# modelstreaming/ams

Measured on AMD Instinct MI355X. Metric: frames/sec student infer (DeeplabV3+MobileNetV2, 512x1024) + distill-steps/sec, higher is better.
Workload: dtype f32 (2xfp16 split products)

## Files before the change

ams_amd/csrc/api.hip:

```cpp
#include "engine.hpp"
#include "head_common.hpp"
#include "entry_check.hpp"

using namespace ams;

extern "C" {

const char* ams_last_error(void) { return ams::last_error(); }
int ams_abi_version(void) { return AMS_ABI_VERSION; }

int ams_device_info(char* name_out, size_t name_cap, int32_t* n_cu, int64_t* hbm_bytes) {
    int dev = 0;
    AMS_CHECK_HIP(hipGetDevice(&dev));
    hipDeviceProp_t p;
    AMS_CHECK_HIP(hipGetDeviceProperties(&p, dev));
    if (name_out && name_cap) { snprintf(name_out, name_cap, "%s (%s)", p.name, p.gcnArchName); }
    if (n_cu) *n_cu = p.multiProcessorCount;
    if (hbm_bytes) *hbm_bytes = (int64_t)p.totalGlobalMem;
    return AMS_OK;
}

int ams_student_arena_bytes(const ams_student_config* cfg, const ams_layer_desc* layers, size_t* bytes_out) {
    AMS_REQUIRE(bytes_out, "arena_bytes: null output");
    ams_student tmp;
// ... 1084 lines not shown
    const bool f32 = !f16 && Cin <= 32;
    const bool wreg = !f32 && presplit == 2;
    BlockCall c;
    c.B = B; c.H = H; c.W = W; c.Cin = Cin; c.Cexp = Cexp; c.rate = rate;
    if (f32 && rate < 0) { c.stride = -rate; c.rate = 1; }
    AMS_REQUIRE(B > 0 && H > 0 && W > 0, "expand_dw_steps: no pixels: B=%d, %d x %d", B, H, W);
    AMS_REQUIRE(expand_dw_stream_supported(Cin, Cexp, c.stride, c.rate) && (!f16 || Cin >= 64), "expand_dw_steps: unsupported shape Cin=%d Cexp=%d rate=%d",
                Cin, Cexp, rate);
    AMS_REQUIRE(out && n >= 10, "expand_dw_steps: out needs at least 10 elements");
    const int np = f32 ? 0 : (f16 ? 2 : 3);
    XdwGeom g;
    const bool fits = wreg ? expand_dw_wreg_geom(B, H, W, Cin, Cexp, c.rate, np, &g) : expand_dw_stream_geom(B, H, W, Cin, Cexp, c.rate, np, &g);
    AMS_REQUIRE(fits, "expand_dw_steps: no segment geometry fits LDS (W=%d rate=%d)", W, rate);
    expand_dw_steps(g, H, W, c.rate, out, n);
    return AMS_OK;
}

int ams_k_global_mean(const float* x, int32_t B, int64_t HW, int32_t C, float* y, float* scratch, size_t scratch_floats,
                      void* stream) {
    AMS_REQUIRE(scratch && scratch_floats >= image_colsum_scratch(B, C), "global_mean: scratch too small (need %zu floats)",
                image_colsum_scratch(B, C));
    return launch_global_mean(x, B, HW, C, y, scratch, (hipStream_t)stream);
}
size_t ams_k_global_mean_scratch(int32_t B, int32_t C) { return image_colsum_scratch(B, C); }

int ams_k_upsample_argmax(const float* logits, int32_t B, int32_t h, int32_t w, int32_t NC, const int32_t* class_idx_host, int32_t K,
                          int32_t H, int32_t W, const uint8_t* teacher, int32_t* labels_out, int64_t* conf_mat, double* loss,
                          void* stream) {
    const HeadCall c{logits, NC, B, h, w, class_idx_host, K, H, W, teacher, NC};
    return launch_upsample_argmax(c, labels_out, conf_mat, loss, (hipStream_t)stream);
// ... 599 lines not shown
```

ams_amd/csrc/k_block.hip:

```cpp
#include <type_traits>

#include "pw_common.hpp"
#include "split_bf16.hpp"
#include "block_call.hpp"

namespace ams {

struct BlkArgs {
    const float* x;
    int B, H, W, Cin;
    const float* w_exp;
    const float* sc_e; const float* sh_e;
    int Cexp;
    const float* w_dw;
    const float* sc_d; const float* sh_d;
    const float* w_pj;
    const float* sc_p; const float* sh_p;
    int Cout;
    int act_e, act_d, act_p, residual;
    float* y;
    int Ho, Wo, pt, pl;
    int tiles_x, tiles_y, chunks;
    const float* vecs;
    int fH, fW, spt, spl;
    float ps;
    const uint16_t* wparts;
    int64_t wplane;
    const uint16_t* he; int64_t he_plane;
    const uint16_t* hp; int64_t hp_plane; int kp_p;
    int timed;
};

__device__ unsigned long long g_blk_cycles[1024][8];

template <typename TIn>
__device__ __forceinline__ float blk_frame_value(const TIn* img, int H, int W, int iy, int ix, int ch, float ps) {
    const bool inside = iy >= 0 && ix >= 0 && iy <= H && ix <= W;
// ... 16 lines not shown

template <int S, int KC, int NTO, int TH, int TW, typename TIn = void, bool X6 = false, bool H16 = false, bool HP = H16>
__global__ __launch_bounds__(256, 2) void block_kernel(BlkArgs a, unsigned ntiles) {
    static_assert(!HP || H16, "HP is a refinement of H16");
    constexpr bool PKDW = S == 1 || TH == 2;
    constexpr bool SLIDE = S == 1 && TW == 16 && TH % 2 == 0;
    constexpr bool STEM = !std::is_void<TIn>::value;
    static_assert(!(X6 && STEM) && !(H16 && STEM) && !(X6 && H16), "the stem stays exact f32; one split form at a time");
    constexpr bool H16W = H16 && KC == 2;
    constexpr int IH = (TH - 1) * S + 3, IW = (TW - 1) * S + 3;
    constexpr int NPIX = IH * IW;
    constexpr int NRG = (NPIX + 15) / 16;
    constexpr int AP = blk_act_pitch(S, TW);
    constexpr int MRO = TH * TW / 16;
    static_assert(TH * TW % 16 == 0, "whole output row groups");
    extern __shared__ __attribute__((aligned(16))) float smem[];
    float* sVec = smem;
    const int tid = threadIdx.x, wave = __builtin_amdgcn_readfirstlane(tid >> 6), lane = tid & 63, l15 = lane & 15, q = lane >> 4;
    float* sAct = smem + 13 * a.Cexp + wave * (NRG * 16 * AP);
    unsigned long long tc[4] = {0, 0, 0, 0}, tl_ = a.timed ? __builtin_amdgcn_s_memtime() : 0;
    auto lap = [&](int slot) {
        if (a.timed) {
            const unsigned long long now = __builtin_amdgcn_s_memtime();
            tc[slot] += now - tl_;
            tl_ = now;
        }
    };

    if (a.vecs) {
        for (int e = tid; e < 13 * a.Cexp / 4; e += 256) st4(sVec + 4 * e, ld4(a.vecs + 4 * e));
    } else {
        for (int e = tid; e < 13 * a.Cexp; e += 256) {
            const int which = e / a.Cexp, c = e - which * a.Cexp;
            const float* src = which == 0 ? a.sc_e : which == 1 ? a.sh_e : which == 2 ? a.sc_d : which == 3 ? a.sh_d : a.w_dw + (which - 4) * a.Cexp;
            sVec[e] = src[c];
        }
    }
    unsigned wt = xcd_remap(blockIdx.x, gridDim.x) * 4 + wave;
    const bool live = wt < ntiles;
    if (!live) wt = ntiles - 1;
    const int tx = wt % a.tiles_x;
    unsigned t1 = wt / a.tiles_x;
    const int ty = t1 % a.tiles_y;
    const int b = t1 / a.tiles_y;
    const int oy0 = ty * TH, ox0 = tx * TW;
    const int iy0 = oy0 * S - a.pt, ix0 = ox0 * S - a.pl;

    const float lo_e = a.act_e == AMS_ACT_NONE ? -__builtin_huge_valf() : 0.f, hi_e = a.act_e == AMS_ACT_RELU6 ? 6.f : __builtin_huge_valf();
    const float lo_d = a.act_d == AMS_ACT_NONE ? -__builtin_huge_valf() : 0.f, hi_d = a.act_d == AMS_ACT_RELU6 ? 6.f : __builtin_huge_valf();
    const float* xb = STEM ? nullptr : a.x + (int64_t)b * a.H * a.W * a.Cin;
    float4 areg[(X6 || H16) ? 1 : NRG][KC];
    bf16x8 xp[X6 ? NRG : 1][3];
    u32x4 xh8[H16W ? NRG : 1], xl8[H16W ? NRG : 1];
    u32x2_t xh4[(H16 && !H16W) ? NRG : 1], xl4[(H16 && !H16W) ? NRG : 1];
    unsigned inside_mask = 0;
    if constexpr (STEM) {
        typedef typename std::conditional<STEM, TIn, float>::type TI;
        const TI* img = reinterpret_cast<const TI*>(a.x) + (int64_t)b * a.fH * a.fW * 3;
        int toff[KC][4], tdy[KC][4], tdx[KC][4], tch[KC][4];
#pragma unroll
        for (int c = 0; c < KC; ++c)
// ... 28 lines not shown
                for (int c = 0; c < KC; ++c)
#pragma unroll
                    for (int j = 0; j < 4; ++j)
                        t[c][j] = blk_frame_value(img, a.fH, a.fW, fy + tdy[c][j], fx + tdx[c][j], tch[c][j] < 0 ? 0 : tch[c][j], a.ps);
            }
#pragma unroll
            for (int c = 0; c < KC; ++c)
                areg[rg][c] = make_float4(tch[c][0] >= 0 ? t[c][0] : 0.f, tch[c][1] >= 0 ? t[c][1] : 0.f, tch[c][2] >= 0 ? t[c][2] : 0.f,
                                          tch[c][3] >= 0 ? t[c][3] : 0.f);
        }
    } else {
#pragma unroll
    for (int rg = 0; rg < NRG; ++rg) {
        const int m = rg * 16 + l15;
        const int ty_i = m / IW, tx_i = m - ty_i * IW;
        const int iy = iy0 + ty_i, ix = ix0 + tx_i;
        if (m < NPIX && iy >= 0 && iy < a.H && ix >= 0 && ix < a.W) inside_mask |= 1u << rg;
        const int iyc = iy < 0 ? 0 : (iy > a.H - 1 ? a.H - 1 : iy), ixc = ix < 0 ? 0 : (ix > a.W - 1 ? a.W - 1 : ix);
        const float* px = xb + ((int64_t)iyc * a.W + ixc) * a.Cin;
        if constexpr (X6 || H16W) {
            int k0 = 8 * q, k1 = 8 * q + 4;
            const bool ok0 = k0 < a.Cin, ok1 = k1 < a.Cin;
            if (k0 > a.Cin - 4) k0 = a.Cin - 4;
            if (k1 > a.Cin - 4) k1 = a.Cin - 4;
            float4 u = ld4(px + k0), v = ld4(px + k1);
            u = make_float4(ok0 ? u.x : 0.f, ok0 ? u.y : 0.f, ok0 ? u.z : 0.f, ok0 ? u.w : 0.f);
            v = make_float4(ok1 ? v.x : 0.f, ok1 ? v.y : 0.f, ok1 ? v.z : 0.f, ok1 ? v.w : 0.f);
            if constexpr (X6) split8(u, v, xp[rg][0], xp[rg][1], xp[rg][2]);
            else {
                f16x8 h, l;
                split8_f16(u, v, h, l);
                xh8[rg] = __builtin_bit_cast(u32x4, h); xl8[rg] = __builtin_bit_cast(u32x4, l);
            }
        } else if constexpr (H16) {
// ... 82 lines not shown
#pragma unroll
        for (int t = 0; t < NTO; ++t) out[i][t] = (f32x4){0.f, 0.f, 0.f, 0.f};
#pragma unroll
    for (int i = 0; i < (HP ? MRO : 1); ++i)
#pragma unroll
        for (int t = 0; t < (HP ? NTO : 1); ++t) outx[i][t] = (f32x4){0.f, 0.f, 0.f, 0.f};
    __syncthreads();
    lap(0);

    const int chunks = a.Cexp / 16;
    for (int ci = 0; ci < chunks; ++ci) {
        const int n0 = ci * 16;
        const int n_next = ci + 1 < chunks ? n0 + 16 : n0;
        {
            const float4 sc = ld4(sVec + n0 + 4 * q), sh = ld4(sVec + a.Cexp + n0 + 4 * q);
#pragma unroll
            for (int rg = 0; rg < NRG; ++rg) {
                f32x4 acc = (f32x4){0.f, 0.f, 0.f, 0.f};
                if constexpr (X6) {
                    acc = __builtin_amdgcn_mfma_f32_16x16x32_bf16(wq[2], xp[rg][0], acc, 0, 0, 0);
                    acc = __builtin_amdgcn_mfma_f32_16x16x32_bf16(wq[0], xp[rg][2], acc, 0, 0, 0);
                    acc = __builtin_amdgcn_mfma_f32_16x16x32_bf16(wq[1], xp[rg][1], acc, 0, 0, 0);
                    acc = __builtin_amdgcn_mfma_f32_16x16x32_bf16(wq[1], xp[rg][0], acc, 0, 0, 0);
                    acc = __builtin_amdgcn_mfma_f32_16x16x32_bf16(wq[0], xp[rg][1], acc, 0, 0, 0);
                    acc = __builtin_amdgcn_mfma_f32_16x16x32_bf16(wq[0], xp[rg][0], acc, 0, 0, 0);
                } else if constexpr (H16) {
                    f32x4 accx = (f32x4){0.f, 0.f, 0.f, 0.f};
                    if constexpr (H16W) {
                        accx = __builtin_amdgcn_mfma_f32_16x16x32_f16(__builtin_bit_cast(f16x8, wl8), __builtin_bit_cast(f16x8, xh8[rg]), accx, 0, 0, 0);
                        accx = __builtin_amdgcn_mfma_f32_16x16x32_f16(__builtin_bit_cast(f16x8, wh8), __builtin_bit_cast(f16x8, xl8[rg]), accx, 0, 0, 0);
                        acc = __builtin_amdgcn_mfma_f32_16x16x32_f16(__builtin_bit_cast(f16x8, wh8), __builtin_bit_cast(f16x8, xh8[rg]), acc, 0, 0, 0);
                    } else {
// ... 8 lines not shown
                        acc = __builtin_amdgcn_mfma_f32_16x16x4f32(wa[c][0], areg[rg][c].x, acc, 0, 0, 0);
                        acc = __builtin_amdgcn_mfma_f32_16x16x4f32(wa[c][1], areg[rg][c].y, acc, 0, 0, 0);
                        acc = __builtin_amdgcn_mfma_f32_16x16x4f32(wa[c][2], areg[rg][c].z, acc, 0, 0, 0);
                        acc = __builtin_amdgcn_mfma_f32_16x16x4f32(wa[c][3], areg[rg][c].w, acc, 0, 0, 0);
                    }
                }
                const bool inside = (inside_mask >> rg) & 1u;
                const float lo = inside ? lo_e : 0.f, hi = inside ? hi_e : 0.f;
                float4 v;
                const float4 bn = muladd4_pk(make_float4(acc[0], acc[1], acc[2], acc[3]), sc, sh);
                v.x = __builtin_amdgcn_fmed3f(bn.x, lo, hi);
                v.y = __builtin_amdgcn_fmed3f(bn.y, lo, hi);
                v.z = __builtin_amdgcn_fmed3f(bn.z, lo, hi);
                v.w = __builtin_amdgcn_fmed3f(bn.w, lo, hi);
                st4(sAct + (rg * 16 + l15) * AP + 4 * q, v);
            }
        }
        load_wa(n_next);
        __builtin_amdgcn_fence(__ATOMIC_RELEASE, "wavefront");
        __builtin_amdgcn_wave_barrier();
        __builtin_amdgcn_fence(__ATOMIC_ACQUIRE, "wavefront");
        lap(1);

        {
            float4 w9[9];
#pragma unroll
            for (int tp = 0; tp < 9; ++tp) w9[tp] = ld4(sVec + (4 + tp) * a.Cexp + n0 + 4 * q);
            const float4 scd = ld4(sVec + 2 * a.Cexp + n0 + 4 * q), shd = ld4(sVec + 3 * a.Cexp + n0 + 4 * q);
            auto finish = [&](int i, const float4& acc) {
                float dv[4];
// ... 6 lines not shown
                    split4_f16(make_float4(dv[0], dv[1], dv[2], dv[3]), h, l);
                    const u32x2_t dh = {h[0], h[1]}, dl = {l[0], l[1]};
#pragma unroll
                    for (int t = 0; t < NTO; ++t) outx[i][t] = mma16_f16(pl[t], dh, outx[i][t]);
#pragma unroll
                    for (int t = 0; t < NTO; ++t) outx[i][t] = mma16_f16(ph[t], dl, outx[i][t]);
#pragma unroll
                    for (int t = 0; t < NTO; ++t) out[i][t] = mma16_f16(ph[t], dh, out[i][t]);
                } else {
#pragma unroll
                    for (int j = 0; j < 4; ++j)
#pragma unroll
                        for (int t = 0; t < NTO; ++t) out[i][t] = __builtin_amdgcn_mfma_f32_16x16x4f32(wp[j][t], dv[j], out[i][t], 0, 0, 0);
                }
            };
            if constexpr (SLIDE) {
                const float* col = sAct + l15 * AP + 4 * q;
                float4 acc[MRO];
#pragma unroll
                for (int i = 0; i < MRO; ++i) acc[i] = make_float4(0.f, 0.f, 0.f, 0.f);
#pragma unroll
                for (int u0 = 0; u0 < TH + 2; u0 += 2) {
                    float4 r[2][3];
#pragma unroll
                    for (int uu = 0; uu < 2; ++uu)
#pragma unroll
                        for (int jj = 0; jj < 3; ++jj) r[uu][jj] = ld4(col + ((u0 + uu) * IW + jj) * AP);
                    asm volatile("" ::: "memory");
#pragma unroll
                    for (int uu = 0; uu < 2; ++uu) {
                        const int u = u0 + uu;
#pragma unroll
                        for (int ii = 0; ii < 3; ++ii) {
                            const int i = u - ii;
                            if (i >= 0 && i < MRO) {
#pragma unroll
                                for (int jj = 0; jj < 3; ++jj) fma4_pk(acc[i], r[uu][jj], w9[ii * 3 + jj]);
                            }
                        }
                        if (u >= 2) finish(u - 2, acc[u - 2]);
                    }
                }
            } else {
#pragma unroll
            for (int i = 0; i < MRO; ++i) {
                const int P = i * 16 + l15;
                const int ly = P / TW, lx = P - ly * TW;
                const float* tap0 = sAct + ((ly * S) * IW + lx * S) * AP + 4 * q;
                float4 tp9[9];
#pragma unroll
                for (int ii = 0; ii < 3; ++ii)
#pragma unroll
                    for (int jj = 0; jj < 3; ++jj) tp9[ii * 3 + jj] = ld4(tap0 + (ii * IW + jj) * AP);
                asm volatile("" ::: "memory");
                float4 acc = make_float4(0.f, 0.f, 0.f, 0.f);
#pragma unroll
                for (int k = 0; k < 9; ++k) {
                    if (PKDW) fma4_pk(acc, tp9[k], w9[k]);
                    else {
                        acc.x = fmaf(tp9[k].x, w9[k].x, acc.x); acc.y = fmaf(tp9[k].y, w9[k].y, acc.y);
                        acc.z = fmaf(tp9[k].z, w9[k].z, acc.z); acc.w = fmaf(tp9[k].w, w9[k].w, acc.w);
                    }
                }
                finish(i, acc);
            }
            }
        }
        load_wp(n_next);
        __builtin_amdgcn_fence(__ATOMIC_RELEASE, "wavefront");
        __builtin_amdgcn_wave_barrier();
        __builtin_amdgcn_fence(__ATOMIC_ACQUIRE, "wavefront");
        lap(2);
    }

    float* yb = a.y + (int64_t)b * a.Ho * a.Wo * a.Cout;
    float4 scp[NTO], shp[NTO], rres[(!STEM) ? MRO : 1][(!STEM) ? NTO : 1];
#pragma unroll
    for (int t = 0; t < NTO; ++t) {
        const int c4 = 16 * t + 4 * q < a.Cout ? 16 * t + 4 * q : 0;
        scp[t] = ld4(a.sc_p + c4);
        shp[t] = ld4(a.sh_p + c4);
    }
    if constexpr (!STEM) {
        if (a.residual) {
#pragma unroll
            for (int i = 0; i < MRO; ++i) {
                const int P = i * 16 + l15;
                const int ly = P / TW, lx = P - ly * TW;
                const int oy = oy0 + ly < a.Ho ? oy0 + ly : a.Ho - 1, ox = ox0 + lx < a.Wo ? ox0 + lx : a.Wo - 1;
#pragma unroll
                for (int t = 0; t < NTO; ++t) rres[i][t] = ld4(xb + ((int64_t)oy * a.W + ox) * a.Cin + (16 * t + 4 * q < a.Cout ? 16 * t + 4 * q : 0));
            }
        }
    }
#pragma unroll
    for (int i = 0; i < MRO; ++i) {
        const int P = i * 16 + l15;
        const int ly = P / TW, lx = P - ly * TW;
        const int oy = oy0 + ly, ox = ox0 + lx;
        if (!live || oy >= a.Ho || ox >= a.Wo) continue;
#pragma unroll
        for (int t = 0; t < NTO; ++t) {
            const int c4 = 16 * t + 4 * q;
            if (c4 >= a.Cout) continue;
            float4 v;
            if constexpr (HP) out[i][t] = combine_f16(out[i][t], outx[HP ? i : 0][HP ? t : 0]);
            const float4 bn = muladd4_pk(make_float4(out[i][t][0], out[i][t][1], out[i][t][2], out[i][t][3]), scp[t], shp[t]);
            v.x = apply_act(bn.x, a.act_p); v.y = apply_act(bn.y, a.act_p);
            v.z = apply_act(bn.z, a.act_p); v.w = apply_act(bn.w, a.act_p);
            if constexpr (!STEM) {
                if (a.residual) {
                    const float4 r = rres[i][t];
                    v.x += r.x; v.y += r.y; v.z += r.z; v.w += r.w;
                }
            }
            st4(yb + ((int64_t)oy * a.Wo + ox) * a.Cout + c4, v);
        }
    }
    if (a.timed) {
        lap(3);
        if (lane == 0) {
            unsigned long long* row = g_blk_cycles[(blockIdx.x * 4 + wave) & 1023];
            for (int i = 0; i < 4; ++i) atomicAdd(&row[i], tc[i]);
            atomicAdd(&row[6], 1ull);
        }
    }
}

template <int S, int KC, int NTO, int TH, int TW, typename TIn = void, bool X6 = false, bool H16 = false, bool HP = H16>
static int launch_blk_k(BlkArgs a, hipStream_t st) {
    constexpr int IH = (TH - 1) * S + 3, IW = (TW - 1) * S + 3;
    constexpr int NRG = (IH * IW + 15) / 16;
    a.tiles_x = cdiv(a.Wo, TW);
    a.tiles_y = cdiv(a.Ho, TH);
    const size_t lds = ((size_t)13 * a.Cexp + (size_t)4 * NRG * 16 * blk_act_pitch(S, TW)) * sizeof(float);
    AMS_REQUIRE(lds <= 64 * 1024, "block kernel: needs %zu bytes of LDS", lds);
    const int64_t ntiles = (int64_t)a.tiles_x * a.tiles_y * a.B;
    const int64_t nblocks = cdiv64(ntiles, 4);
    AMS_REQUIRE(ntiles > 0 && ntiles < 0x7fffffffLL, "block kernel: bad grid");
    static const std::string nm = "block_kernel<" + std::to_string(S) + ", " + std::to_string(KC) + ", " + std::to_string(NTO) + ", " +
                                  std::to_string(TH) + ", " + std::to_string(TW) +
                                  (std::is_void<TIn>::value ? ", void" : sizeof(typename std::conditional<std::is_void<TIn>::value, char, TIn>::type) == 1 ? ", unsigned char" : ", float") +
                                  (X6 ? ", true" : ", false") + (H16 ? ", true" : ", false") + (HP ? ", true>" : ", false>");
    note_kernel(nm.c_str());
    hipLaunchKernelGGL((block_kernel<S, KC, NTO, TH, TW, TIn, X6, H16, HP>), dim3((unsigned)nblocks), dim3(256), lds, st, a, (unsigned)ntiles);
    AMS_CHECK_LAUNCH();
    return AMS_OK;
}

template <int S, int TH, int TW>
static int launch_blk_t(const BlkArgs& a, hipStream_t st) {
    const bool k1 = (a.Cin + 15) / 16 == 1, o2 = a.Cout <= 32;
// ... 69 lines not shown
    else if (c.expand.np && c.Cin > 16) { a.wparts = c.expand.panels; a.wplane = c.expand.plane; }
    same_pad(c.H, 3, stride, 1, &a.Ho, &a.pt);
    same_pad(c.W, 3, stride, 1, &a.Wo, &a.pl);
    int th, tw;
    AMS_REQUIRE(blk_pick_tile(Cexp, Cout, stride, a.wparts != nullptr || a.he != nullptr, &th, &tw), "block kernel: no tile fits LDS for Cexp=%d", Cexp);
    if (knobs().blk_th > 0 && blk_lds_bytes(stride, knobs().blk_th, knobs().blk_tw, Cexp) <= 64 * 1024) {
        th = knobs().blk_th; tw = knobs().blk_tw;
    }
#define BLK(S_, TH_, TW_) if (stride == S_ && th == TH_ && tw == TW_) return launch_blk_t<S_, TH_, TW_>(a, st);
    BLK(1, 8, 8) BLK(1, 4, 16) BLK(1, 4, 8) BLK(2, 4, 8) BLK(2, 2, 8) BLK(2, 4, 4)
#undef BLK
    set_error("block kernel: no %dx%d tile for stride %d", th, tw, stride);
    return AMS_E_INVALID;
}

int launch_first_block_tiles(const BlockCall& c, hipStream_t st) {
    RUN_RC(block_call_check("first_block_tiles", BK_FIRST_TILES, c));
    BlkArgs a;
    memset(&a, 0, sizeof(a));
    a.x = reinterpret_cast<const float*>(c.frames); a.B = c.B; a.fH = c.H; a.fW = c.W; a.ps = c.pixel_scale; a.Cin = 27;
    blk_layers(c, &a);
    same_pad(c.H + 1, 3, 2, 1, &a.H, &a.spt);
    same_pad(c.W + 1, 3, 2, 1, &a.W, &a.spl);
    a.Ho = a.H; a.Wo = a.W; a.pt = 1; a.pl = 1;
    if (c.dtype == AMS_DT_U8) return launch_blk_k<1, 2, 1, 8, 8, uint8_t>(a, st);
    return launch_blk_k<1, 2, 1, 8, 8, float>(a, st);
}

int blk_phase_cycles(unsigned long long* h) {
    static unsigned long long rows[1024][8], z[1024][8];
// ... 10 lines not shown
```

ams_amd/csrc/kernels.hpp:

```cpp
#pragma once
#include <vector>

#include "common.hpp"

struct ams_comm;

namespace ams {

struct ConvLayer;
struct BlockCall;

int func_allow_lds(const void* fn, size_t lds);
int func_blocks_per_cu(const void* fn, int threads, size_t lds, int* per_cu);
int device_cus(int* cus);
bool launch_table_needs_attr(int device, const void* fn, size_t lds);
struct Knobs {
    int blk_th = 0, blk_tw = 0;
    int fb_walk = -1;
    int fb_abl = 0;
    int xwr_timed = 0;
    int blk_timed = 0;
    int blk_hp = -1;
    char pw_force = 0; int pw_rm = 0, pw_nt = 0;
    int pw_percu = 0;
    bool pwx_no_tail = false;
    int pwx_rm = 0, pwx_nt = 0;
    int xwr_abl = 0;
    int pwh_abl = 0;
    bool pwh_set = false; int pwh_nw = 4, pwh_d = 2;
    bool xds_set = false; int xds[6] = {0, 0, 0, 0, 0, 0};
    bool xwr_set = false; int xwr[5] = {0, 0, 0, 0, 0};
    bool wg6_eight_waves = false;
    int wg6_split_cap = 0;
    int event_flags = -1;
    unsigned side_cu_mask = 0;
};
const Knobs& knobs();
// ... 148 lines not shown
                      int act_e, const float* w_dw, int stride, const float* dz_d, const float* cA, const float* cB, const float* cC,
                      const float* res, float* dx, hipStream_t st, const float* red_z = nullptr, const float* red_mean = nullptr,
                      const float* red_rstd = nullptr, float* red_part = nullptr, int* red_rows_out = nullptr);
int launch_xdw_dwe(const float* G1, const float* xx_g0, int Cin, int Cexp, const float* w_exp, const float* cA, const float* cB, const float* cC,
                   float* dw, hipStream_t st);

int xx_stats_blocks(int64_t M);
size_t xx_stats_scratch_doubles(int64_t M, int Cin);
int launch_xx_gram(const float* x, int64_t M, int Cin, double* scratch, double* xx64, float* xx32, hipStream_t st);
int launch_expand_stats(const double* xx64, int Cin, const float* w_exp, int Cexp, double n, const float* center, const float* gamma,
                        const float* beta, float eps, float one_minus_decay, float* moving_mean, float* moving_var, float* scale, float* shift,
                        float* save_mean, float* save_rstd, double* sums, hipStream_t st);

bool block_fused_supported(int Cin, int Cexp, int Cout, int stride, int rate, bool residual);
int launch_block_fused(const BlockCall& c, hipStream_t st);
int launch_first_block_tiles(const BlockCall& c, hipStream_t st);
int launch_block_pack(const float* sc_e, const float* sh_e, const float* sc_d, const float* sh_d, const float* w_dw, int Cexp, float* out, hipStream_t st);

constexpr int AMS_NP_F16 = 4;
bool expand_dw_stream_supported(int Cin, int Cexp, int stride, int rate);
int launch_expand_dw_stream(const BlockCall& c, hipStream_t st);

int launch_expand_dw_wreg(const BlockCall& c, hipStream_t st);
struct XdwGeom { int step, SH, SW, Wp, T, ring, nsy, nsx, cgroups, items, groups, nt, nwe, nwd, nrg; size_t lds; };
bool expand_dw_stream_geom(int B, int H, int W, int Cin, int Cexp, int rate, int np, XdwGeom* g);
bool expand_dw_wreg_geom(int B, int H, int W, int Cin, int Cexp, int rate, int np, XdwGeom* g);
void expand_dw_steps(const XdwGeom& g, int H, int W, int rate, int32_t* out, size_t n);


size_t image_colsum_scratch(int B, int C);
// ... 150 lines not shown
```

ams_amd/csrc/runtime.hip:

```cpp
#include <stdlib.h>

#include <map>
#include <mutex>
#include <tuple>

#include "kernels.hpp"

namespace ams {

namespace {
std::mutex g_mu;
std::map<std::pair<int, const void*>, size_t> g_attr;
std::map<std::tuple<int, const void*, int, size_t>, int> g_occ;
std::map<int, int> g_cus;
}

bool launch_table_needs_attr(int device, const void* fn, size_t lds) {
    std::lock_guard<std::mutex> lk(g_mu);
    size_t& have = g_attr[{device, fn}];
    if (lds <= have) return false;
    have = lds;
    return true;
}

// ... 37 lines not shown
        auto it = g_cus.find(dev);
        if (it != g_cus.end()) { *cus = it->second; return AMS_OK; }
    }
    int n = 0;
    AMS_CHECK_HIP(hipDeviceGetAttribute(&n, hipDeviceAttributeMultiprocessorCount, dev));
    std::lock_guard<std::mutex> lk(g_mu);
    g_cus[dev] = n;
    *cus = n;
    return AMS_OK;
}

static Knobs read_knobs() {
        Knobs v;
        if (const char* e = getenv("AMS_BLK_TILE")) sscanf(e, "%dx%d", &v.blk_th, &v.blk_tw);
        if (const char* e = getenv("AMS_BLK_HP")) v.blk_hp = atoi(e);
        if (const char* e = getenv("AMS_FB_WALK")) v.fb_walk = atoi(e);
        if (const char* e = getenv("AMS_BLK_TIMED")) v.blk_timed = atoi(e);
        if (const char* e = getenv("AMS_XWR_TIMED")) v.xwr_timed = atoi(e);
        if (const char* e = getenv("AMS_PW_FORCE")) sscanf(e, "%c,%d,%d", &v.pw_force, &v.pw_rm, &v.pw_nt);
        if (const char* e = getenv("AMS_PW_PERCU")) v.pw_percu = atoi(e);
        v.pwx_no_tail = getenv("AMS_PWX_NO_TAIL") != nullptr;
#ifdef AMS_MEASURE
        if (const char* e = getenv("AMS_FB_ABL")) v.fb_abl = atoi(e);
        if (const char* e = getenv("AMS_PWH_ABL")) v.pwh_abl = atoi(e);
        if (const char* e = getenv("AMS_XWR_ABL")) v.xwr_abl = atoi(e);
#else
        for (const char* name : {"AMS_FB_ABL", "AMS_PWH_ABL", "AMS_XWR_ABL"})
            if (const char* e = getenv(name))
                if (atoi(e) != 0) fprintf(stderr, "libams_hip: %s=%s ignored — ablated kernels exist only in libams_hip_measure.so (make -C ams_amd/csrc measure)\n", name, e);
#endif
// ... 44 lines not shown
```

ams_amd/hip.py:

```python
from __future__ import annotations

import ctypes as C
import os
from pathlib import Path

_HERE = Path(__file__).resolve().parent
LIB_PATH = _HERE / "libams_hip.so"

ABI_VERSION = 6

ROLE_STEM, ROLE_EXPAND, ROLE_DEPTHWISE, ROLE_PROJECT, ROLE_POOL_CONV, ROLE_ASPP, ROLE_CONCAT_PROJ, ROLE_LOGITS = range(8)
ACT_NONE, ACT_RELU, ACT_RELU6 = 0, 1, 2
DT_F32, DT_U8, DT_I32, DT_F64 = 0, 1, 3, 4
MODE_FROZEN, MODE_LIVE = 0, 1
OPT_MATMUL = 1
RESIZE_NEAREST, RESIZE_LINEAR = 0, 1
OPT_FUSE_EXPAND_DW = 2
OPT_FUSE_DW_PROJECT = 3
OPT_FUSE_FIRST_BLOCK = 4
OPT_FUSE_EXPAND_DW_STREAM = 5
OPT_FUSE_BLOCK = 6
OPT_LATE_SUBBATCH = 7
OPT_BLOCK_X6 = 8
OPT_DUAL_STREAM = 10
# ... 150 lines not shown
    "ams_k_pointwise_split": (C.c_int, [_vp, _i64, _i32, _vp, _i32, _vp, _vp, _i32, _vp, _vp, _vp, _sz, _vp]),
    "ams_k_pointwise_split3": (C.c_int, [_vp, _i64, _i32, _vp, _i32, _vp, _vp, _i32, _vp, _vp, _vp, _sz, _vp]),
    "ams_k_pack_h2i": (C.c_int, [_vp, _i64, _i32, _vp, _vp]),
    "ams_k_pointwise_split_f16": (C.c_int, [_vp, _i64, _i32, _vp, _i32, _vp, _vp, _i32, _vp, _vp, _vp, _sz, _vp, _vp, _vp]),
    "ams_k_expand_dw_stream_f16": (C.c_int, [_vp, _i32, _i32, _i32, _i32, _vp, _vp, _vp, _i32, _vp, _i32, _vp, _vp, _vp, _vp, _sz, _i32, _i32, _vp]),
    "ams_ingest_resize_u8": (C.c_int, [_vp, _i32, _i32, _i32, _i32, _i32, _vp, _i32, _i32, _vp]),
    "ams_k_dw_project": (C.c_int, [_vp, _i32, _i32, _i32, _i32, _vp, _i32, _vp, _vp, _vp, _i32, _vp, _vp, _vp, _vp, _vp, _sz, _vp]),
    "ams_k_block_fused": (C.c_int, [_vp, _i32, _i32, _i32, _i32, _vp, _vp, _vp, _i32, _vp, _i32, _vp, _vp, _vp, _i32, _vp, _vp, _i32, _vp, _vp, _sz, _vp]),
    "ams_k_block_fused_f16": (C.c_int, [_vp, _i32, _i32, _i32, _i32, _vp, _vp, _vp, _i32, _vp, _i32, _vp, _vp, _vp, _i32, _vp, _vp, _i32, _vp, _vp, _sz, _vp]),
    "ams_k_first_block_scratch": (_sz, [_i32]),
    "ams_k_first_block": (C.c_int, [_vp, _i32, _i32, _i32, _i32, _f32, _vp, _vp, _vp, _vp, _vp, _vp, _vp, _vp, _vp, _vp, _i32, _vp, _sz,
                                    C.POINTER(FirstBlockPlan), _vp]),
    "ams_k_first_block_tiles": (C.c_int, [_vp, _i32, _i32, _i32, _i32, _f32, _vp, _vp, _vp, _vp, _vp, _vp, _vp, _vp, _vp, _vp, _vp]),
    "ams_k_first_block_plan": (C.c_int, [_i32, _i32, _i32, _i32, _i32, C.POINTER(_i32), C.POINTER(FirstBlockPlan)]),
    "ams_k_expand_dw_steps": (C.c_int, [_i32, _i32, _i32, _i32, _i32, _i32, _i32, _i32, C.POINTER(_i32), _sz]),
    "ams_k_expand_dw": (C.c_int, [_vp, _i32, _i32, _i32, _i32, _vp, _vp, _vp, _i32, _vp, _i32, _i32, _vp, _vp, _vp, _vp]),
    "ams_k_expand_dw_stream": (C.c_int, [_vp, _i32, _i32, _i32, _i32, _vp, _vp, _vp, _i32, _vp, _i32, _vp, _vp, _vp, _vp, _sz, _i32, _i32, _vp]),
    "ams_k_global_mean": (C.c_int, [_vp, _i32, _i64, _i32, _vp, _vp, _sz, _vp]),
    "ams_k_global_mean_scratch": (_sz, [_i32, _i32]),
    "ams_k_upsample_argmax": (C.c_int, [_vp, _i32, _i32, _i32, _i32, C.POINTER(_i32), _i32, _i32, _i32, _vp, _vp, _vp,
                                        _vp, _vp]),
    "ams_k_upsample_confidence": (C.c_int, [_vp, _i32, _i32, _i32, _i32, C.POINTER(_i32), _i32, _i32, _i32, _vp, _vp, _vp, _vp, _vp]),
    "ams_confidence_stats_len": (_sz, []),
    "ams_k_upsample_soft_metric": (C.c_int, [_vp, _i32, _i32, _i32, _i32, C.POINTER(_i32), _i32, _i32, _i32, _vp, _vp, _i32, _i32, _vp, _vp, _vp, _vp]),
    "ams_k_upsample_soft_metric_layout": (C.c_int, [_vp, _i32, _i32, _i32, _i32, _i32, C.POINTER(_i32), _i32, _i32, _i32, _vp, _vp, _i32, _i32, _i32, _vp, _vp, _vp, _vp]),
    "ams_soft_metric_stats_len": (_sz, [_i32]),
    "ams_k_ce_grad": (C.c_int, [_vp, _i32, _i32, _i32, _i32, C.POINTER(_i32), _i32, _i32, _i32, _vp, _vp, _vp, _vp]),
    "ams_k_ce_loss_grad": (C.c_int, [_vp, _i32, _i32, _i32, _i32, C.POINTER(_i32), _i32, _i32, _i32, _vp, _vp, _vp, _vp, _sz, _vp]),
    "ams_k_ce_loss_grad_scratch": (_sz, [_i32, _i32, _i32, _i32]),
    "ams_k_ce_loss_grad_soft": (C.c_int, [_vp, _i32, _i32, _i32, _i32, C.POINTER(_i32), _i32, _i32, _i32, _vp, _vp, _i32, _i32, _vp, _vp, _vp, _sz, _vp]),
# ... 103 lines not shown
```

include/ams_hip.h:

```cpp
#ifndef AMS_HIP_H
#define AMS_HIP_H

#include <stddef.h>
#include <stdint.h>

#ifdef __cplusplus
extern "C" {
#endif

#define AMS_ABI_VERSION 6

enum {
    AMS_OK = 0,
    AMS_E_INVALID = -1,
    AMS_E_HIP = -2,
    AMS_E_STATE = -3,
    AMS_E_NOMEM = -4
};

enum {
    AMS_ROLE_STEM = 0,
    AMS_ROLE_EXPAND = 1,
    AMS_ROLE_DEPTHWISE = 2,
    AMS_ROLE_PROJECT = 3,
// ... 364 lines not shown
    int32_t interior_tiles, interior_grid;
    int32_t border_tiles, border_grid;
    int32_t border_walks;
} ams_first_block_plan;
size_t ams_k_first_block_scratch(int32_t form);
int ams_k_first_block(const void* frames, int32_t frames_dtype, int32_t B, int32_t H, int32_t W, float pixel_scale, const float* w_stem,
                      const float* scale_s, const float* shift_s, const float* w_dw, const float* scale_d, const float* shift_d, const float* w_proj,
                      const float* scale_p, const float* shift_p, float* y, int32_t form, uint16_t* panels, size_t panel_elems,
                      ams_first_block_plan* plan_out, void* stream);
int ams_k_first_block_tiles(const void* frames, int32_t frames_dtype, int32_t B, int32_t H, int32_t W, float pixel_scale, const float* w_stem,
                            const float* scale_s, const float* shift_s, const float* w_dw, const float* scale_d, const float* shift_d,
                            const float* w_proj, const float* scale_p, const float* shift_p, float* y, void* stream);
int ams_k_first_block_plan(int32_t frames_dtype, int32_t B, int32_t H, int32_t W, int32_t form, const int32_t* occupancy, ams_first_block_plan* plan_out);
int ams_k_expand_dw_steps(int32_t B, int32_t H, int32_t W, int32_t Cin, int32_t Cexp, int32_t rate, int32_t f16, int32_t presplit, int32_t* out,
                          size_t n);

enum { AMS_RESIZE_NEAREST = 0, AMS_RESIZE_LINEAR = 1 };
int ams_ingest_resize_u8(const uint8_t* src, int32_t Hs, int32_t Ws, int32_t C, int32_t mode, int32_t swap_rb, uint8_t* dst,
                         int32_t H, int32_t W, void* stream);

int ams_k_global_mean(const float* x, int32_t B, int64_t HW, int32_t C, float* y, float* scratch, size_t scratch_floats,
                      void* stream);
size_t ams_k_global_mean_scratch(int32_t B, int32_t C);

int ams_k_upsample_argmax(const float* logits , int32_t B, int32_t h, int32_t w, int32_t NC,
                          const int32_t* class_idx_host, int32_t K, int32_t H, int32_t W, const uint8_t* teacher,
                          int32_t* labels_out, int64_t* conf_mat, double* loss, void* stream);

#define AMS_CONFIDENCE_BINS 32
int ams_k_upsample_confidence(const float* logits , int32_t B, int32_t h, int32_t w, int32_t NC,
// ... 159 lines not shown
```

Before: 12870.

## Transpose ragged edge tiles and skip dead row groups in fused block kernel

Fused block tiling gains an edge-aware scheme. A narrow remainder column of width at most TH is covered by transposed tiles rather than mostly-empty regular tiles. Tiles cut off at the bottom skip expand row groups and depthwise output groups that hold no valid rows. Both are on by default through a new env knob, and a host API exposes the tile walk for inspection. The aim is to cut wasted MFMA and LDS work on partial tiles, at the cost of runtime index arithmetic, strided addressing in the transposed path and per-tile branching in the inner loops.

```diff
diff --git a/ams_amd/csrc/api.hip b/ams_amd/csrc/api.hip
--- a/ams_amd/csrc/api.hip
+++ b/ams_amd/csrc/api.hip
@@ -1122,6 +1122,10 @@
     AMS_REQUIRE(fits, "expand_dw_steps: no segment geometry fits LDS (W=%d rate=%d)", W, rate);
     expand_dw_steps(g, H, W, c.rate, out, n);
     return AMS_OK;
+}
+
+int ams_k_block_tiles(int32_t B, int32_t Ho, int32_t Wo, int32_t stride, int32_t th, int32_t tw, int32_t* out, size_t n) {
+    return block_tiles_walk(B, Ho, Wo, stride, th, tw, out, n);
 }
 
 int ams_k_global_mean(const float* x, int32_t B, int64_t HW, int32_t C, float* y, float* scratch, size_t scratch_floats,
diff --git a/ams_amd/csrc/blk_tiles.hpp b/ams_amd/csrc/blk_tiles.hpp
--- /dev/null
+++ b/ams_amd/csrc/blk_tiles.hpp
@@ -0,0 +1,66 @@
+#pragma once
+
+#if defined(__HIPCC__) || defined(__CUDACC__)
+#define AMS_BLK_HD __host__ __device__ inline
+#else
+#define AMS_BLK_HD inline
+#endif
+
+namespace ams {
+
+enum BlkTileClass { BLK_TILE_REGULAR = 0, BLK_TILE_TRANSPOSED = 1 };
+enum BlkEdge { BLK_EDGE_TRANSPOSE = 1, BLK_EDGE_SKIP = 2 };
+
+struct BlkTiling {
+    int Ho, Wo, TH, TW;
+    int rw;
+    int nx, ny;
+    int nreg, ntr;
+    int skip;
+};
+
+AMS_BLK_HD constexpr bool blk_form_transposes(int S, int TH, int TW) { return !(S == 1 && TW == 16 && TH % 2 == 0); }
+
+AMS_BLK_HD BlkTiling blk_tiling(int S, int Ho, int Wo, int TH, int TW, int edge) {
+    BlkTiling g;
+    g.Ho = Ho; g.Wo = Wo; g.TH = TH; g.TW = TW;
+    const int rw = Wo % TW;
+    g.rw = (edge & BLK_EDGE_TRANSPOSE) && blk_form_transposes(S, TH, TW) && rw > 0 && rw <= TH ? rw : 0;
+    g.nx = g.rw ? Wo / TW : (Wo + TW - 1) / TW;
+    g.ny = (Ho + TH - 1) / TH;
+    g.nreg = g.nx * g.ny;
+    g.ntr = g.rw ? (Ho + TW - 1) / TW : 0;
+    g.skip = (edge & BLK_EDGE_SKIP) ? 1 : 0;
+    return g;
+}
+
+struct BlkTile { int b, oy0, ox0, cls, vh, vw; };
+
+AMS_BLK_HD BlkTile blk_tile(const BlkTiling& g, unsigned index) {
+    const unsigned per_frame = (unsigned)(g.nreg + g.ntr);
+    BlkTile t;
+    t.b = (int)(index / per_frame);
+    const int r = (int)(index - (unsigned)t.b * per_frame);
+    if (r < g.nreg) {
+        const int ty = r / (g.nx > 0 ? g.nx : 1), tx = r - ty * g.nx;
+        t.cls = BLK_TILE_REGULAR;
+        t.oy0 = ty * g.TH; t.ox0 = tx * g.TW;
+        t.vh = g.Ho - t.oy0 < g.TH ? g.Ho - t.oy0 : g.TH;
+        const int wreg = g.Wo - g.rw;
+        t.vw = wreg - t.ox0 < g.TW ? wreg - t.ox0 : g.TW;
+    } else {
+        t.cls = BLK_TILE_TRANSPOSED;
+        t.oy0 = (r - g.nreg) * g.TW; t.ox0 = g.Wo - g.rw;
+        t.vh = g.rw;
+        t.vw = g.Ho - t.oy0 < g.TW ? g.Ho - t.oy0 : g.TW;
+    }
+    return t;
+}
+
+AMS_BLK_HD int blk_expand_groups(int vh, int S, int IW, int nrg) {
+    const int need = (((vh - 1) * S + 3) * IW + 15) / 16;
+    return need < nrg ? need : nrg;
+}
+AMS_BLK_HD bool blk_output_group_live(int i, int vh, int TW) { return i * 16 / TW < vh; }
+
+}
diff --git a/ams_amd/csrc/k_block.hip b/ams_amd/csrc/k_block.hip
--- a/ams_amd/csrc/k_block.hip
+++ b/ams_amd/csrc/k_block.hip
@@ -3,6 +3,7 @@
 #include "pw_common.hpp"
 #include "split_bf16.hpp"
 #include "block_call.hpp"
+#include "blk_tiles.hpp"
 
 namespace ams {
 
@@ -20,7 +21,8 @@
     int act_e, act_d, act_p, residual;
     float* y;
     int Ho, Wo, pt, pl;
-    int tiles_x, tiles_y, chunks;
+    BlkTiling tl;
+    int chunks;
     const float* vecs;
     int fH, fW, spt, spl;
     float ps;
@@ -67,6 +69,7 @@
     constexpr int AP = blk_act_pitch(S, TW);
     constexpr int MRO = TH * TW / 16;
     static_assert(TH * TW % 16 == 0, "whole output row groups");
+    static_assert(!(SLIDE && blk_form_transposes(S, TH, TW)), "the sliding taps have no transposed form");
     extern __shared__ __attribute__((aligned(16))) float smem[];
     float* sVec = smem;
     const int tid = threadIdx.x, wave = __builtin_amdgcn_readfirstlane(tid >> 6), lane = tid & 63, l15 = lane & 15, q = lane >> 4;
@@ -92,12 +95,15 @@
     unsigned wt = xcd_remap(blockIdx.x, gridDim.x) * 4 + wave;
     const bool live = wt < ntiles;
     if (!live) wt = ntiles - 1;
-    const int tx = wt % a.tiles_x;
-    unsigned t1 = wt / a.tiles_x;
-    const int ty = t1 % a.tiles_y;
-    const int b = t1 / a.tiles_y;
-    const int oy0 = ty * TH, ox0 = tx * TW;
+    const BlkTile tile = blk_tile(a.tl, wt);
+    const int b = tile.b, oy0 = tile.oy0, ox0 = tile.ox0;
+    const bool tr = !blk_form_transposes(S, TH, TW) || STEM ? false : __builtin_amdgcn_readfirstlane(tile.cls) == BLK_TILE_TRANSPOSED;
+    const int vh = STEM ? TH : __builtin_amdgcn_readfirstlane(a.tl.skip ? tile.vh : TH);
     const int iy0 = oy0 * S - a.pt, ix0 = ox0 * S - a.pl;
+    const int g0 = tr ? ix0 : iy0, g1 = tr ? iy0 : ix0, n0i = tr ? a.W : a.H, n1i = tr ? a.H : a.W;
+    const int64_t xrow = (int64_t)a.W * a.Cin, yrow = (int64_t)a.Wo * a.Cout;
+    const int64_t xs0 = tr ? (int64_t)a.Cin : xrow, xs1 = tr ? xrow : (int64_t)a.Cin, ys0 = tr ? (int64_t)a.Cout : yrow, ys1 = tr ? yrow : (int64_t)a.Cout;
+    const int e0 = tr ? ox0 : oy0, e1 = tr ? oy0 : ox0, n0o = tr ? a.Wo : a.Ho, n1o = tr ? a.Ho : a.Wo;
 
     const float lo_e = a.act_e == AMS_ACT_NONE ? -__builtin_huge_valf() : 0.f, hi_e = a.act_e == AMS_ACT_RELU6 ? 6.f : __builtin_huge_valf();
     const float lo_d = a.act_d == AMS_ACT_NONE ? -__builtin_huge_valf() : 0.f, hi_d = a.act_d == AMS_ACT_RELU6 ? 6.f : __builtin_huge_valf();
@@ -156,10 +162,10 @@
     for (int rg = 0; rg < NRG; ++rg) {
         const int m = rg * 16 + l15;
         const int ty_i = m / IW, tx_i = m - ty_i * IW;
-        const int iy = iy0 + ty_i, ix = ix0 + tx_i;
-        if (m < NPIX && iy >= 0 && iy < a.H && ix >= 0 && ix < a.W) inside_mask |= 1u << rg;
-        const int iyc = iy < 0 ? 0 : (iy > a.H - 1 ? a.H - 1 : iy), ixc = ix < 0 ? 0 : (ix > a.W - 1 ? a.W - 1 : ix);
-        const float* px = xb + ((int64_t)iyc * a.W + ixc) * a.Cin;
+        const int iy = g0 + ty_i, ix = g1 + tx_i;
+        if (m < NPIX && iy >= 0 && iy < n0i && ix >= 0 && ix < n1i) inside_mask |= 1u << rg;
+        const int iyc = iy < 0 ? 0 : (iy > n0i - 1 ? n0i - 1 : iy), ixc = ix < 0 ? 0 : (ix > n1i - 1 ? n1i - 1 : ix);
+        const float* px = xb + (iyc * xs0 + ixc * xs1);
         if constexpr (X6 || H16W) {
             int k0 = 8 * q, k1 = 8 * q + 4;
             const bool ok0 = k0 < a.Cin, ok1 = k1 < a.Cin;
@@ -272,8 +278,7 @@
         const int n_next = ci + 1 < chunks ? n0 + 16 : n0;
         {
             const float4 sc = ld4(sVec + n0 + 4 * q), sh = ld4(sVec + a.Cexp + n0 + 4 * q);
-#pragma unroll
-            for (int rg = 0; rg < NRG; ++rg) {
+            auto expand_rg = [&](int rg) {
                 f32x4 acc = (f32x4){0.f, 0.f, 0.f, 0.f};
                 if constexpr (X6) {
                     acc = __builtin_amdgcn_mfma_f32_16x16x32_bf16(wq[2], xp[rg][0], acc, 0, 0, 0);
@@ -312,6 +317,13 @@
                 v.z = __builtin_amdgcn_fmed3f(bn.z, lo, hi);
                 v.w = __builtin_amdgcn_fmed3f(bn.w, lo, hi);
                 st4(sAct + (rg * 16 + l15) * AP + 4 * q, v);
+            };
+#pragma unroll
+            for (int v = 1; v <= TH; ++v) {
+                if (v > 1 && v > vh) continue;
+#pragma unroll
+                for (int rg = 0; rg < NRG; ++rg)
+                    if (rg >= (v == 1 ? 0 : blk_expand_groups(v - 1, S, IW, NRG)) && rg < blk_expand_groups(v, S, IW, NRG)) expand_rg(rg);
             }
         }
         load_wa(n_next);
@@ -348,36 +360,8 @@
                         for (int t = 0; t < NTO; ++t) out[i][t] = __builtin_amdgcn_mfma_f32_16x16x4f32(wp[j][t], dv[j], out[i][t], 0, 0, 0);
                 }
             };
-            if constexpr (SLIDE) {
-                const float* col = sAct + l15 * AP + 4 * q;
-                float4 acc[MRO];
-#pragma unroll
-                for (int i = 0; i < MRO; ++i) acc[i] = make_float4(0.f, 0.f, 0.f, 0.f);
-#pragma unroll
-                for (int u0 = 0; u0 < TH + 2; u0 += 2) {
-                    float4 r[2][3];
-#pragma unroll
-                    for (int uu = 0; uu < 2; ++uu)
-#pragma unroll
-                        for (int jj = 0; jj < 3; ++jj) r[uu][jj] = ld4(col + ((u0 + uu) * IW + jj) * AP);
-                    asm volatile("" ::: "memory");
-#pragma unroll
-                    for (int uu = 0; uu < 2; ++uu) {
-                        const int u = u0 + uu;
-#pragma unroll
-                        for (int ii = 0; ii < 3; ++ii) {
-                            const int i = u - ii;
-                            if (i >= 0 && i < MRO) {
-#pragma unroll
-                                for (int jj = 0; jj < 3; ++jj) fma4_pk(acc[i], r[uu][jj], w9[ii * 3 + jj]);
-                            }
-                        }
-                        if (u >= 2) finish(u - 2, acc[u - 2]);
-                    }
-                }
-            } else {
-#pragma unroll
-            for (int i = 0; i < MRO; ++i) {
+            auto nine_taps = [&](int i, auto trc) {
+                constexpr bool TR = decltype(trc)::value;
                 const int P = i * 16 + l15;
                 const int ly = P / TW, lx = P - ly * TW;
                 const float* tap0 = sAct + ((ly * S) * IW + lx * S) * AP + 4 * q;
@@ -385,7 +369,7 @@
 #pragma unroll
                 for (int ii = 0; ii < 3; ++ii)
 #pragma unroll
-                    for (int jj = 0; jj < 3; ++jj) tp9[ii * 3 + jj] = ld4(tap0 + (ii * IW + jj) * AP);
+                    for (int jj = 0; jj < 3; ++jj) tp9[ii * 3 + jj] = ld4(tap0 + (TR ? jj * IW + ii : ii * IW + jj) * AP);
                 asm volatile("" ::: "memory");
                 float4 acc = make_float4(0.f, 0.f, 0.f, 0.f);
 #pragma unroll
@@ -396,9 +380,49 @@
                         acc.z = fmaf(tp9[k].z, w9[k].z, acc.z); acc.w = fmaf(tp9[k].w, w9[k].w, acc.w);
                     }
                 }
-                finish(i, acc);
-            }
-            }
+                return acc;
+            };
+            auto by_groups = [&](auto) {
+#pragma unroll
+                for (int i = 0; i < MRO; ++i) {
+                    if (i > 0 && !blk_output_group_live(i, vh, TW)) continue;
+                    float4 acc;
+                    if (tr) acc = nine_taps(i, std::true_type());
+                    else acc = nine_taps(i, std::false_type());
+                    finish(i, acc);
+                }
+            };
+            auto slide = [&](auto) {
+                const float* col = sAct + l15 * AP + 4 * q;
+                float4 acc[MRO];
+#pragma unroll
+                for (int i = 0; i < MRO; ++i) acc[i] = make_float4(0.f, 0.f, 0.f, 0.f);
+#pragma unroll
+                for (int u0 = 0; u0 < TH + 2; u0 += 2) {
+                    if (u0 >= 2 && u0 >= vh + 2) continue;
+                    float4 r[2][3];
+#pragma unroll
+                    for (int uu = 0; uu < 2; ++uu)
+#pragma unroll
+                        for (int jj = 0; jj < 3; ++jj) r[uu][jj] = ld4(col + ((u0 + uu) * IW + jj) * AP);
+                    asm volatile("" ::: "memory");
+#pragma unroll
+                    for (int uu = 0; uu < 2; ++uu) {
+                        const int u = u0 + uu;
+#pragma unroll
+                        for (int ii = 0; ii < 3; ++ii) {
+                            const int i = u - ii;
+                            if (i >= 0 && i < MRO) {
+#pragma unroll
+                                for (int jj = 0; jj < 3; ++jj) fma4_pk(acc[i], r[uu][jj], w9[ii * 3 + jj]);
+                            }
+                        }
+                        if (u >= 2 && (u == 2 || u - 2 < vh)) finish(u - 2, acc[u - 2]);
+                    }
+                }
+            };
+            if constexpr (SLIDE) slide(0);
+            else by_groups(0);
         }
         load_wp(n_next);
         __builtin_amdgcn_fence(__ATOMIC_RELEASE, "wavefront");
@@ -421,9 +445,9 @@
             for (int i = 0; i < MRO; ++i) {
                 const int P = i * 16 + l15;
                 const int ly = P / TW, lx = P - ly * TW;
-                const int oy = oy0 + ly < a.Ho ? oy0 + ly : a.Ho - 1, ox = ox0 + lx < a.Wo ? ox0 + lx : a.Wo - 1;
-#pragma unroll
-                for (int t = 0; t < NTO; ++t) rres[i][t] = ld4(xb + ((int64_t)oy * a.W + ox) * a.Cin + (16 * t + 4 * q < a.Cout ? 16 * t + 4 * q : 0));
+                const int oy = e0 + ly < n0o ? e0 + ly : n0o - 1, ox = e1 + lx < n1o ? e1 + lx : n1o - 1;
+#pragma unroll
+                for (int t = 0; t < NTO; ++t) rres[i][t] = ld4(xb + (oy * xs0 + ox * xs1) + (16 * t + 4 * q < a.Cout ? 16 * t + 4 * q : 0));
             }
         }
     }
@@ -431,8 +455,8 @@
     for (int i = 0; i < MRO; ++i) {
         const int P = i * 16 + l15;
         const int ly = P / TW, lx = P - ly * TW;
-        const int oy = oy0 + ly, ox = ox0 + lx;
-        if (!live || oy >= a.Ho || ox >= a.Wo) continue;
+        const int oy = e0 + ly, ox = e1 + lx;
+        if (!live || oy >= n0o || ox >= n1o) continue;
 #pragma unroll
         for (int t = 0; t < NTO; ++t) {
             const int c4 = 16 * t + 4 * q;
@@ -448,7 +472,7 @@
                     v.x += r.x; v.y += r.y; v.z += r.z; v.w += r.w;
                 }
             }
-            st4(yb + ((int64_t)oy * a.Wo + ox) * a.Cout + c4, v);
+            st4(yb + (oy * ys0 + ox * ys1) + c4, v);
         }
     }
     if (a.timed) {
@@ -465,11 +489,10 @@
 static int launch_blk_k(BlkArgs a, hipStream_t st) {
     constexpr int IH = (TH - 1) * S + 3, IW = (TW - 1) * S + 3;
     constexpr int NRG = (IH * IW + 15) / 16;
-    a.tiles_x = cdiv(a.Wo, TW);
-    a.tiles_y = cdiv(a.Ho, TH);
+    a.tl = blk_tiling(S, a.Ho, a.Wo, TH, TW, std::is_void<TIn>::value ? knobs().blk_edge : 0);
     const size_t lds = ((size_t)13 * a.Cexp + (size_t)4 * NRG * 16 * blk_act_pitch(S, TW)) * sizeof(float);
     AMS_REQUIRE(lds <= 64 * 1024, "block kernel: needs %zu bytes of LDS", lds);
-    const int64_t ntiles = (int64_t)a.tiles_x * a.tiles_y * a.B;
+    const int64_t ntiles = (int64_t)(a.tl.nreg + a.tl.ntr) * a.B;
     const int64_t nblocks = cdiv64(ntiles, 4);
     AMS_REQUIRE(ntiles > 0 && ntiles < 0x7fffffffLL, "block kernel: bad grid");
     static const std::string nm = "block_kernel<" + std::to_string(S) + ", " + std::to_string(KC) + ", " + std::to_string(NTO) + ", " +
@@ -569,6 +592,31 @@
     return AMS_E_INVALID;
 }
 
+int block_tiles_walk(int B, int Ho, int Wo, int stride, int th, int tw, int32_t* out, size_t n) {
+    AMS_REQUIRE(B > 0 && Ho > 0 && Wo > 0, "block_tiles: no pixels: B=%d, %d x %d", B, Ho, Wo);
+    bool known = false;
+#define BLK(S_, TH_, TW_) known = known || (stride == S_ && th == TH_ && tw == TW_);
+    BLK(1, 8, 8) BLK(1, 4, 16) BLK(1, 4, 8) BLK(2, 4, 8) BLK(2, 2, 8) BLK(2, 4, 4)
+#undef BLK
+    AMS_REQUIRE(known, "block_tiles: no %dx%d tile for stride %d", th, tw, stride);
+    AMS_REQUIRE(out && n >= 8, "block_tiles: out needs at least 8 elements");
+    const BlkTiling g = blk_tiling(stride, Ho, Wo, th, tw, knobs().blk_edge);
+    const int ih = (th - 1) * stride + 3, iw = (tw - 1) * stride + 3;
+    const int nrg = (ih * iw + 15) / 16, mro = th * tw / 16;
+    const int64_t ntiles = (int64_t)(g.nreg + g.ntr) * B;
+    AMS_REQUIRE(ntiles < 0x7fffffffLL, "block_tiles: bad grid");
+    out[0] = g.nx; out[1] = g.ny; out[2] = g.nreg; out[3] = g.ntr; out[4] = g.rw; out[5] = (int32_t)ntiles; out[6] = nrg; out[7] = mro;
+    for (int64_t i = 0; i < ntiles && 8 + 8 * (size_t)(i + 1) <= n; ++i) {
+        const BlkTile t = blk_tile(g, (unsigned)i);
+        const int vh = g.skip ? t.vh : th;
+        int live = 0;
+        for (int r = 0; r < mro; ++r) live += r == 0 || blk_output_group_live(r, vh, tw);
+        int32_t* o = out + 8 + 8 * i;
+        o[0] = t.b; o[1] = t.oy0; o[2] = t.ox0; o[3] = t.cls; o[4] = t.vh; o[5] = t.vw; o[6] = blk_expand_groups(vh, stride, iw, nrg); o[7] = live;
+    }
+    return AMS_OK;
+}
+
 int launch_first_block_tiles(const BlockCall& c, hipStream_t st) {
     RUN_RC(block_call_check("first_block_tiles", BK_FIRST_TILES, c));
     BlkArgs a;
diff --git a/ams_amd/csrc/kernels.hpp b/ams_amd/csrc/kernels.hpp
--- a/ams_amd/csrc/kernels.hpp
+++ b/ams_amd/csrc/kernels.hpp
@@ -21,6 +21,7 @@
     int xwr_timed = 0;
     int blk_timed = 0;
     int blk_hp = -1;
+    int blk_edge = 3;
     char pw_force = 0; int pw_rm = 0, pw_nt = 0;
     int pw_percu = 0;
     bool pwx_no_tail = false;
@@ -199,6 +200,7 @@
 
 bool block_fused_supported(int Cin, int Cexp, int Cout, int stride, int rate, bool residual);
 int launch_block_fused(const BlockCall& c, hipStream_t st);
+int block_tiles_walk(int B, int Ho, int Wo, int stride, int th, int tw, int32_t* out, size_t n);
 int launch_first_block_tiles(const BlockCall& c, hipStream_t st);
 int launch_block_pack(const float* sc_e, const float* sh_e, const float* sc_d, const float* sh_d, const float* w_dw, int Cexp, float* out, hipStream_t st);
 
diff --git a/ams_amd/csrc/runtime.hip b/ams_amd/csrc/runtime.hip
--- a/ams_amd/csrc/runtime.hip
+++ b/ams_amd/csrc/runtime.hip
@@ -75,6 +75,7 @@
         Knobs v;
         if (const char* e = getenv("AMS_BLK_TILE")) sscanf(e, "%dx%d", &v.blk_th, &v.blk_tw);
         if (const char* e = getenv("AMS_BLK_HP")) v.blk_hp = atoi(e);
+        if (const char* e = getenv("AMS_BLK_EDGE")) v.blk_edge = atoi(e) & 3;
         if (const char* e = getenv("AMS_FB_WALK")) v.fb_walk = atoi(e);
         if (const char* e = getenv("AMS_BLK_TIMED")) v.blk_timed = atoi(e);
         if (const char* e = getenv("AMS_XWR_TIMED")) v.xwr_timed = atoi(e);
diff --git a/ams_amd/hip.py b/ams_amd/hip.py
--- a/ams_amd/hip.py
+++ b/ams_amd/hip.py
@@ -188,6 +188,7 @@
     "ams_k_first_block_tiles": (C.c_int, [_vp, _i32, _i32, _i32, _i32, _f32, _vp, _vp, _vp, _vp, _vp, _vp, _vp, _vp, _vp, _vp, _vp]),
     "ams_k_first_block_plan": (C.c_int, [_i32, _i32, _i32, _i32, _i32, C.POINTER(_i32), C.POINTER(FirstBlockPlan)]),
     "ams_k_expand_dw_steps": (C.c_int, [_i32, _i32, _i32, _i32, _i32, _i32, _i32, _i32, C.POINTER(_i32), _sz]),
+    "ams_k_block_tiles": (C.c_int, [_i32, _i32, _i32, _i32, _i32, _i32, C.POINTER(_i32), _sz]),
     "ams_k_expand_dw": (C.c_int, [_vp, _i32, _i32, _i32, _i32, _vp, _vp, _vp, _i32, _vp, _i32, _i32, _vp, _vp, _vp, _vp]),
     "ams_k_expand_dw_stream": (C.c_int, [_vp, _i32, _i32, _i32, _i32, _vp, _vp, _vp, _i32, _vp, _i32, _vp, _vp, _vp, _vp, _sz, _i32, _i32, _vp]),
     "ams_k_global_mean": (C.c_int, [_vp, _i32, _i64, _i32, _vp, _vp, _sz, _vp]),
diff --git a/include/ams_hip.h b/include/ams_hip.h
--- a/include/ams_hip.h
+++ b/include/ams_hip.h
@@ -402,6 +402,7 @@
 int ams_k_first_block_plan(int32_t frames_dtype, int32_t B, int32_t H, int32_t W, int32_t form, const int32_t* occupancy, ams_first_block_plan* plan_out);
 int ams_k_expand_dw_steps(int32_t B, int32_t H, int32_t W, int32_t Cin, int32_t Cexp, int32_t rate, int32_t f16, int32_t presplit, int32_t* out,
                           size_t n);
+int ams_k_block_tiles(int32_t B, int32_t Ho, int32_t Wo, int32_t stride, int32_t th, int32_t tw, int32_t* out, size_t n);
 
 enum { AMS_RESIZE_NEAREST = 0, AMS_RESIZE_LINEAR = 1 };
 int ams_ingest_resize_u8(const uint8_t* src, int32_t Hs, int32_t Ws, int32_t C, int32_t mode, int32_t swap_rb, uint8_t* dst,
```

Measured after the change: 12790. No clear change (-0.7%).
